# cartographer-project/cartographer

Hardware: AMD Instinct MI355X
Metric: candidate poses scored/sec (higher is better)
Workload: dtype u8/int32; 1 GPU; C2: 2D FastCorrelativeScanMatcher MatchFullSubmap (branch and bound): 1000-point scan vs 1 400x400 submap(s) per GPU, depth 7, full-angle search, m...; submaps_per_gpu=1, rotations=2373, found=1

## Files before the change

cartographer_amd/csrc/cmx_common.h:

```cpp
#ifndef CMX_COMMON_H_
#define CMX_COMMON_H_

#include <hip/hip_runtime.h>

#include <cstdarg>
#include <cstdint>
#include <cstdio>
#include <cstring>
#include <functional>
#include <mutex>
#include <string>
#include <vector>

#include "../../include/cartographer_mi355x.h"

namespace cmx {

void SetLastError(const char* fmt, ...);
const char* LastError();

struct HipError {
  cmx_status status;
};

#define CMX_HIP(expr)                                                              \
  do {                                                                             \
    hipError_t cmx_err__ = (expr);                                                 \
    if (cmx_err__ != hipSuccess) {                                                 \
      ::cmx::SetLastError("%s failed: %s (%s:%d)", #expr,                          \
                          hipGetErrorString(cmx_err__), __FILE__, __LINE__);       \
      throw ::cmx::HipError{cmx_err__ == hipErrorOutOfMemory ? CMX_OUT_OF_MEMORY   \
                                                             : CMX_DEVICE_ERROR};  \
    }                                                                              \
  } while (0)

#define CMX_REQUIRE(cond, ...)                       \
  do {                                               \
    if (!(cond)) {                                   \
      ::cmx::SetLastError(__VA_ARGS__);              \
      throw ::cmx::HipError{CMX_INVALID_ARGUMENT};   \
    }                                                \
  } while (0)

template <typename F>
cmx_status Guard(F&& body) {
  try {
    body();
    return CMX_OK;
  } catch (const HipError& e) {
    return e.status;
  } catch (const std::bad_alloc&) {
    SetLastError("host allocation failed");
    return CMX_OUT_OF_MEMORY;
  } catch (const std::exception& e) {
    SetLastError("exception: %s", e.what());
    return CMX_DEVICE_ERROR;
  }
}

#define CMX_DEBUG_OPTIONS(X)                                                                      \
  X(rt2d_legacy)                 \
  X(rt2d_tile)                                        \
  X(rt2d_groups)                                   \
  X(rt2d_target)                                    \
  X(rt2d_lds_kb)                                         \
  X(rt2d_no_image_cache)             \
  X(rt2d_parts)                                 \
  X(rt2d_host_par)         \
  X(rt2d_tables_serial)    \
  X(rt2d_first_part)       \
  X(rt2d_image_kernels)    \
  X(rt2d_no_lane)          \
  X(rt2d_parts_pool)       \
  X(rt2d_grid_share)       \
  X(rt2d_unfused)            \
  X(rt2d_no_bounds)        \
  X(rt2d_bounds)           \
  X(rt2d_bounds_fused)     \
  X(rt2d_bounds_level)     \
  X(rt2d_bounds_verify)    \
  X(rt2d_tsdf_batch_legacy)  \
  X(rt2d_tsdf_batch_bulk)  \
  X(rt2d_tsdf_verify)      \
  X(timeline)                  \
  X(trace)                       \
  X(host_trace)                          \
  X(launch_serial)         \
  X(sync)                      \
  X(no_copy_kernels)             \
  X(timing)                \
  X(no_direct_results)     \
  X(frontier_capacity)     \
  X(comm_virtual_ranks)    \
  X(comm_force_rccl)       \
  X(fast2d_unfused)                    \
  X(fast2d_store_scans)                   \
  X(fast2d_fused_threads)                            \
  X(fast2d_fanout)         \
  X(fast2d_group)          \
  X(fast2d_group_verify)   \
  X(fast2d_levels_per_stage)                                    \
  X(fast2d_wave_levels)                        \
  X(fast2d_xcd_affinity)                          \
  X(fast2d_dive)           \
  X(fast2d_queue)          \
  X(fast2d_queue_blocks)                \
  X(fast2d_queue_capacity)              \
  X(fast2d_queue_lost)       \
  X(filters_generic)       \
  X(fast3d_byte_loads)                             \
  X(fast3d_affinity)                              \
  X(fast3d_no_families)                             \
  X(fast3d_no_oct)                                         \
  X(fast3d_batch)                                                 \
  X(fast3d_chunk_cells)    \
  X(rt3d_legacy)                  \
  X(rt3d_no_tiles)                      \
  X(rt3d_verify)                  \
  X(rt3d_no_rotblocks)              \
  X(rt3d_rotblock_permille)  \
  X(rt3d_crosscheck)           \
  X(rt3d_expand_all)       \
  X(rt3d_unstaged)                                     \
  X(rt3d_no_boxes)                            \
  X(rt3d_report)                                             \
  X(rt3d_segments)                         \
  X(rt3d_group_rotations)                                  \
  X(rt3d_group_tile_kb)                                   \
  X(rt3d_group_float)                          \
  X(rt3d_cand_threads)                                   \
  X(rt3d_cand_rotations)                                    \
  X(rt3d_cand_tile_kb)
struct DebugOptions {
#define CMX_DEBUG_FIELD(name) int name = 0;
  CMX_DEBUG_OPTIONS(CMX_DEBUG_FIELD)
#undef CMX_DEBUG_FIELD
};
const DebugOptions& Debug();
bool DebugSet(const char* name, int value);

void UseDevice(int device);

void ParallelFor(int n, int serial_below, const std::function<void(int)>& fn);

class LaunchTurn {
 public:
  LaunchTurn();
  ~LaunchTurn();
  LaunchTurn(const LaunchTurn&) = delete;
  LaunchTurn& operator=(const LaunchTurn&) = delete;
 private:
  bool held_;
};

class HostLane {
 public:
  HostLane();
  ~HostLane();
  HostLane(const HostLane&) = delete;
  HostLane& operator=(const HostLane&) = delete;
  void Run(std::function<void()> fn);
  void Wait();
  bool own() const { return own_; }

 private:
  bool own_ = false, pending_ = false;
};

class DeviceBuffer {
 public:
  DeviceBuffer() = default;
  DeviceBuffer(const DeviceBuffer&) = delete;
  DeviceBuffer& operator=(const DeviceBuffer&) = delete;
  ~DeviceBuffer() { Free(); }
  void* Reserve(size_t bytes) {
    if (bytes > capacity_) {
      Free();
      const size_t want = bytes + bytes / 4 + 256;
      CMX_HIP(hipMalloc(&ptr_, want));
      capacity_ = want;
    }
    return ptr_;
  }
  template <typename T>
  T* ReserveAs(size_t count) { return static_cast<T*>(Reserve(count * sizeof(T))); }
  void* get() const { return ptr_; }
  size_t capacity() const { return capacity_; }
// ... 131 lines not shown
```

cartographer_amd/csrc/fast_2d.hip:

```cpp
#include <algorithm>
#include <chrono>
#include <cstring>
#include <memory>
#include <type_traits>
#include <utility>

#include "fast_2d_device.h"
#include "fast_2d_internal.h"

namespace cmx {
namespace {

constexpr int kSeedsPerProblem = 64;

constexpr int kMaxStages = kMaxDepth + 2;

constexpr int kCountStride = 32;
constexpr int kQueues = 2048;
struct alignas(8) QueueCtl {
  int head;
  int reserved;
  int pad[30];
};
struct Counters {
  int frontier[kMaxStages][kSubLists * kCountStride];
  int leaves[kSubLists * kCountStride];
  int frontier_overflow;
  int leaf_overflow;
  unsigned wave_gathers;
  int blocks_done;
  int pad[28];
  unsigned gathers_shard[16 * kCountStride];
  unsigned queue_stats[16 * kCountStride];
  QueueCtl queue[kQueues];
};

struct CountersSummary {
  int leaves[kSubLists];
  int frontier_total[kMaxStages];
  int frontier_overflow;
  int leaf_overflow;
  unsigned wave_gathers;
  int pad;
  unsigned queue_stats[8];
};

struct NodeList {
  Node2D* nodes;
  int* counts;
  int sub_capacity;
};

__device__ __forceinline__ int ListReserve(const NodeList& list, int sub, int m) {
  return atomicAdd(&list.counts[sub * kCountStride], m);
}
__device__ __forceinline__ bool ListStore(const NodeList& list, int sub, int slot,
                                          const Node2D& nd) {
  if (slot >= list.sub_capacity) return false;
  list.nodes[static_cast<size_t>(sub) * list.sub_capacity + slot] = nd;
  return true;
}
__device__ __forceinline__ int ListMaxCount(const NodeList& list) {
  const int lane = threadIdx.x & 63;
  return WaveMax(min(list.counts[lane * kCountStride], list.sub_capacity));
}

__device__ __forceinline__ int NodeProblem(const Node2D& nd) { return nd.problem & 0xffffff; }
__device__ __forceinline__ int NodeLevel(const Node2D& nd) { return nd.problem >> 24; }

__device__ __forceinline__ Node2D CoarseNode(const Fast2DProblem& P, int problem, int s,
                                             int local) {
  const int2 dims = P.coarse_dims[s];
  const int4 bd = P.bounds[s];
  const int step = 1 << (P.depth - 1);
  const int ix = local / dims.y, iy = local - ix * dims.y;
  const int c = s * P.coarse_stride + local;
  Node2D nd;
  nd.problem = problem | ((P.depth - 1) << 24);
  nd.scan = s;
  nd.dx = bd.x + ix * step;
  nd.dy = bd.z + iy * step;
  nd.score = P.coarse_score[c];
  nd.coarse_index = c;
  nd.path = 0;
  nd.coarse_score = nd.score;
  return nd;
}

struct SeedScratch {
  int hist[1024];
  int wave_total[4];
  int threshold_bin;
  int found_scan[4];
  int total;
};

__device__ __forceinline__ void PickSeeds(const Fast2DProblem& P, int n, int want0, int wants,
                                          SeedScratch* sh) {
  const int tid = threadIdx.x, lane = tid & 63, T = blockDim.x;
  for (int i = tid; i < 1024; i += T) sh->hist[i] = 0;
  if (tid < 4) sh->found_scan[tid] = -1;
  if (tid == 0) sh->total = 0;
  __syncthreads();
  const int S = P.num_scans;
  const long long range = 255ll * n + 1;
  const auto* scan_best = AsGlobal(P.scan_best);
  const auto* coarse_dims = AsGlobal(P.coarse_dims);
  const bool grouped = P.group > 1;
  const auto best_of = [&](int s) -> int {
    if (grouped) {
      const int first = s - s % kFusedGroup;
      if (s != first + (S - first >= kFusedGroup ? 1 : 0)) return -1;
    }
    return scan_best[s].x;
  };
  constexpr int kOwn = 16;
  int own[kOwn];
#pragma unroll
  for (int k = 0; k < kOwn; ++k) {
    const int s = tid + k * T;
    own[k] = s < S ? best_of(s) : -1;
  }
  int total = 0;
#pragma unroll
  for (int k = 0; k < kOwn; ++k)
    if (own[k] >= 0) atomicAdd(&sh->hist[static_cast<int>(own[k] * 1024ll / range)], 1);
  for (int s = tid + kOwn * T; s < S; s += T) {
    const int b = best_of(s);
    if (b >= 0) atomicAdd(&sh->hist[static_cast<int>(b * 1024ll / range)], 1);
  }
  if (want0 == 0) {
    for (int s = tid; s < S; s += T) total += coarse_dims[s].x * coarse_dims[s].y;
    total = WaveSum(total);
    if (lane == 0 && total) atomicAdd(&sh->total, total);
  }
  __syncthreads();
  if (tid < 64) {
    int mine = 0;
#pragma unroll
    for (int k = 0; k < 16; ++k) mine += sh->hist[1023 - 16 * lane - k];
    int incl = mine;
#pragma unroll
    for (int off = 1; off < 64; off <<= 1) {
      const int o = __shfl_up(incl, off, 64);
      if (lane >= off) incl += o;
    }
    const unsigned long long reached = __ballot(incl >= kSeedsPerProblem);
    int tb = 0;
    if (reached) {
      const int first = __ffsll(static_cast<long long>(reached)) - 1;
      if (lane == first) {
        int acc = incl - mine;
        for (int k = 0; k < 16; ++k) {
          const int b = 1023 - 16 * lane - k;
          acc += sh->hist[b];
          if (acc >= kSeedsPerProblem) { tb = b; break; }
        }
        sh->threshold_bin = tb;
      }
    } else if (lane == 0) {
      sh->threshold_bin = 0;
    }
  }
  __syncthreads();
  const int tb = sh->threshold_bin;
  const auto qualifies = [&](int best) {
    return best >= 0 && static_cast<int>(best * 1024ll / range) >= tb &&
           ToScore(P, best, n) > P.min_score;
  };
// ... 162 lines not shown
    const int total = sh->partial[0][k] + sh->partial[1][k] + sh->partial[2][k] + sh->partial[3][k];
    const float mine = valid ? ToScoreCtx(ctx, total) : -1.f;
    int rank = 0, nvalid = 0;
#pragma unroll
    for (int j = 0; j < 4; ++j) {
      const float other = __shfl(mine, j, 64);
      if (other >= 0.f) ++nvalid;
      if (j != k && other >= 0.f && (other > mine || (other == mine && j < k))) ++rank;
    }
    if (threadIdx.x < 4) {
      sh->child_score[k] = mine;
      sh->rank[k] = rank;
      if (k == 0) sh->nvalid = nvalid;
    }
  }
  __syncthreads();
}

__device__ __forceinline__ Node2D MakeChild(const Node2D& nd, int k, int child_level,
                                            const ChildScratch& sh) {
  Node2D child = nd;
  child.problem = NodeProblem(nd) | (child_level << 24);
  child.dx = nd.dx + (k >> 1) * (1 << child_level);
  child.dy = nd.dy + (k & 1) * (1 << child_level);
  child.score = sh.child_score[k];
  child.path = nd.path | (static_cast<unsigned>(sh.rank[k]) << (2 * child_level));
  return child;
}

__device__ __forceinline__ void RecordLeaf(const Node2D& leaf, const NodeList& leaves,
                                           Counters* __restrict__ counters) {
  const int sub = blockIdx.x & (kSubLists - 1);
  if (!ListStore(leaves, sub, ListReserve(leaves, sub, 1), leaf)) counters->leaf_overflow = 1;
}

__global__ void __launch_bounds__(256, 4)
DiveKernel(const Fast2DProblem* __restrict__ problems, ProblemState* __restrict__ states, int n,
           NodeList leaves, Counters* __restrict__ counters) {
  const int problem = blockIdx.y;
  const Fast2DProblem& P = problems[problem];
  ProblemState& st = states[problem];
  if (st.error) return;
  __shared__ BlockContext ctx;
  __shared__ ChildScratch sh;
  __shared__ Node2D cur;
  __shared__ SeedScratch seed_scratch;
  const int per_seed = P.group > 1 ? kFusedGroup : 1;
  if (static_cast<int>(blockIdx.x) >= kSeedsPerProblem * per_seed) return;
  int seed_scan;
  const bool have_seed = PickSeed(P, n, blockIdx.x / per_seed, &seed_scratch, &seed_scan);
  if (blockIdx.x == 0 && threadIdx.x == 0) st.coarse_total = seed_scratch.total;
  if (!have_seed) return;
  if (per_seed > 1) {
    seed_scan = seed_scan - seed_scan % kFusedGroup + static_cast<int>(blockIdx.x) % per_seed;
    if (seed_scan >= P.num_scans) return;
  }
  const Node2D seed = CoarseNode(P, problem, seed_scan, P.scan_best[seed_scan].y);
  if (threadIdx.x == 0) cur = seed;
  LoadContext(P, n, seed.scan, &ctx);
  const int depth = NodeLevel(seed) + 1;
  unsigned long long scored = 0;
  for (int child_level = depth - 2; child_level >= 0; --child_level) {
    const Node2D nd = cur;
    ScoreChildren(ctx, nd.dx, nd.dy, child_level, &sh);
    scored += sh.nvalid;
    if (threadIdx.x == 0) {
      for (int k = 0; k < 4; ++k)
        if (sh.child_score[k] >= 0.f && sh.rank[k] == 0) cur = MakeChild(nd, k, child_level, sh);
    }
    __syncthreads();
  }
  if (threadIdx.x == 0) {
    const Node2D leaf = cur;
    if (leaf.score > ctx.min_score) {
      RecordLeaf(leaf, leaves, counters);
      atomicMax(&st.best_bits, __float_as_uint(leaf.score));
    }
    atomicAdd(&st.scored_shard[blockIdx.x & (kStatShards - 1)], scored);
    atomicAdd(&st.expanded_shard[blockIdx.x & (kStatShards - 1)],
              static_cast<unsigned long long>(depth - 1));
  }
}

__global__ void __launch_bounds__(256)
FilterCoarseKernel(const Fast2DProblem* __restrict__ problems,
                   const ProblemState* __restrict__ states, int n, int chunk, int num_chunks,
                   int strict, int affinity, NodeList out, Counters* __restrict__ counters) {
  const int problem = blockIdx.y;
  const Fast2DProblem& P = problems[problem];
  const int lane = threadIdx.x & 63;
  const int s = blockIdx.x * 4 + __builtin_amdgcn_readfirstlane(threadIdx.x >> 6);
  if (s >= P.num_scans || states[problem].error) return;
  if (s % num_chunks != chunk) return;
  const float best = __uint_as_float(states[problem].best_bits);
  const float top = ToScore(P, P.scan_best[s].x, n);
  if (strict ? !(top > best) : (top < best)) return;
  const int2 dims = P.coarse_dims[s];
  const int count = dims.x * dims.y;
  const int base = s * P.coarse_stride;
  const auto* scores = AsGlobal(P.coarse_score) + base;
  float ahead[4];
#pragma unroll
  for (int k = 0; k < 4; ++k) ahead[k] = k * kWave + lane < count ? scores[k * kWave + lane] : 0.f;
  for (int c0 = 0; c0 < count; c0 += kWave) {
    const int sub = affinity ? (problem & 7) + 8 * ((s + (c0 >> 6)) & 7)
                             : (s + blockIdx.y + (c0 >> 6)) & (kSubLists - 1);
    const int c = c0 + lane;
    bool keep = false;
    if (c < count) {
      float score;
      switch (c0 >> 6) {
        case 0: score = ahead[0]; break;
        case 1: score = ahead[1]; break;
        case 2: score = ahead[2]; break;
        case 3: score = ahead[3]; break;
        default: score = scores[c];
      }
      keep = strict ? (score > best) : (score >= best);
    }
    const unsigned long long mask = __ballot(keep);
    if (mask == 0) continue;
    int first = 0;
    if (lane == 0) first = ListReserve(out, sub, __popcll(mask));
    first = __builtin_amdgcn_readfirstlane(first);
    if (keep) {
      const int slot = first + __popcll(mask & ((1ull << lane) - 1));
      if (!ListStore(out, sub, slot, CoarseNode(P, problem, s, c))) counters->frontier_overflow = 1;
    }
  }
}

constexpr int kWaveStatProblems = 1024;

__global__ void __launch_bounds__(256)
ExpandWaveKernel(const Fast2DProblem* __restrict__ problems, ProblemState* __restrict__ states,
                 int n, NodeList in, int strict, int affinity, NodeList out,
                 Counters* __restrict__ counters) {
  __shared__ unsigned stat_scored[kWaveStatProblems], stat_expanded[kWaveStatProblems];
  __shared__ unsigned stat_gathers;
  if (threadIdx.x == 0) stat_gathers = 0;
  for (int i = threadIdx.x; i < kWaveStatProblems; i += blockDim.x) {
    stat_scored[i] = 0;
    stat_expanded[i] = 0;
  }
  __syncthreads();
  const int lane = threadIdx.x & 63;
  const int wave = __builtin_amdgcn_readfirstlane(threadIdx.x >> 6);
  const int max_count = ListMaxCount(in);
  int first = blockIdx.x * 4 + wave;
  if (affinity) {
    const int slot = (blockIdx.x >> 3) * 4 + wave;
    first = (slot >> 3) * kSubLists + (blockIdx.x & 7) + 8 * (slot & 7);
  }
  const int out_sub = first & (kSubLists - 1);
  for (int i = first; i < max_count * kSubLists; i += gridDim.x * 4) {
    const int in_sub = i & (kSubLists - 1), j = i / kSubLists;
    if (j >= in.counts[in_sub * kCountStride]) continue;
    const Node2D nd = in.nodes[static_cast<size_t>(in_sub) * in.sub_capacity + j];
    const int problem = NodeProblem(nd);
    const Fast2DProblem& P = problems[problem];
    ProblemState& st = states[problem];
    const float best = __uint_as_float(st.best_bits);
    if (strict ? !(nd.score > best) : (nd.score < best)) continue;
    const int child_level = NodeLevel(nd) - 1;
    const LevelDesc L = P.level[child_level];
    const int4 bd = P.bounds[nd.scan];
    const int half = 1 << child_level, off = half - 1;
    const bool vx = nd.dx + half <= bd.y, vy = nd.dy + half <= bd.w;
    const auto* pts = AsGlobal(P.discrete) + static_cast<size_t>(nd.scan) * n;
    const bool recompute = P.recompute_scans != 0 && P.store_scans == 0;
    const float2 rot = recompute ? P.scan_rot[nd.scan] : make_float2(1.f, 0.f);
    const int parent_ub = SumUpperBound(P, nd.score, n);
    const unsigned long long quad_bytes =
        static_cast<unsigned long long>((L.qy + 3) >> 2) * static_cast<unsigned>(L.qtx) * 128ull;
    const bool quads_by_buffer = quad_bytes < (1ull << 31);
    const __amdgpu_buffer_rsrc_t quad_rsrc = __builtin_amdgcn_make_buffer_rsrc(
        const_cast<uint32_t*>(L.quads), 0, quads_by_buffer ? static_cast<int>(quad_bytes) : 0,
        0x00020000);
    const auto* quads = AsGlobal(L.quads);
    const uint32_t child_mask =
        (vx ? 0xffffffffu : 0x0000ffffu) & (vy ? 0xffffffffu : 0x00ff00ffu);
    int s00 = 0, s01 = 0, s10 = 0, s11 = 0, seen_max = 0;
    int groups = 0;
    bool dead = false;
    constexpr int kIters = 4;
    constexpr int kGroup = kIters * kWave;
    const auto walk = [&](auto recompute_tag, auto buffer_tag) {
      constexpr bool kRecompute = decltype(recompute_tag)::value;
      constexpr bool kBuffer = decltype(buffer_tag)::value;
      for (int q0 = 0; q0 < n; q0 += kGroup) {
        uint32_t cell[kIters];
#pragma unroll
        for (int u = 0; u < kIters; ++u) {
          const int q = q0 + u * kWave + lane;
          const int at = q < n ? q : 0;
          if constexpr (kRecompute) cell[u] = ScanCell(P, rot, at);
          else cell[u] = pts[at];
        }
        uint32_t v[kIters];
#pragma unroll
        for (int u = 0; u < kIters; ++u) {
          const int q = q0 + u * kWave + lane;
          const bool live = q < n;
          const uint32_t p = cell[u];
          const int X = static_cast<short>(p & 0xffffu) + nd.dx + off + half;
          const int Y = static_cast<short>(p >> 16) + nd.dy + off + half;
          const bool inside = live && static_cast<unsigned>(X) < static_cast<unsigned>(L.qx) &&
                              static_cast<unsigned>(Y) < static_cast<unsigned>(L.qy);
          if constexpr (kBuffer) {
            const uint32_t quad = __builtin_amdgcn_raw_buffer_load_b32(
                quad_rsrc, inside ? QuadOffset(X, Y, L.qtx) * 4u : 0xfffffff0u, 0, 0);
            v[u] = quad & child_mask;
// ... 546 lines not shown
  const int lane = threadIdx.x & 63;
  const auto* pts = AsGlobal(P.discrete) + static_cast<size_t>(scan) * n;
  if constexpr (kRecompute) {
    const float2 rot = P.scan_rot[scan];
#pragma unroll
    for (int u = 0; u < kChainCells; ++u) cell[u] = kNoCell;
#pragma unroll 1
    for (int j = 0; j * kWave < n; ++j) {
      const int i = j * kWave + lane;
      const uint32_t c = i < n ? ScanCell(P, rot, i) : kNoCell;
#pragma unroll
      for (int u = 0; u < kChainCells; ++u) cell[u] = u == j ? c : cell[u];
    }
  } else {
#pragma unroll
    for (int j = 0; j < kChainCells; ++j) {
      const int i = j * kWave + lane;
      cell[j] = kNoCell;
      if (j * kWave < n) cell[j] = i < n ? pts[i] : kNoCell;
    }
  }
}

struct ChainLevel {
  int qx, qy, qtx;
  int half;
  int ax, ay;
  __amdgpu_buffer_rsrc_t quad_rsrc;
};

__device__ __forceinline__ ChainLevel MakeChainLevel(const Fast2DProblem& P, int child_level,
                                                     int dx, int dy) {
  const LevelDesc& Lm = P.level[child_level];
  ChainLevel L;
  L.half = 1 << child_level;
  L.ax = dx + 2 * L.half - 1;
  L.ay = dy + 2 * L.half - 1;
  L.qx = __builtin_amdgcn_readfirstlane(Lm.qx);
  L.qy = __builtin_amdgcn_readfirstlane(Lm.qy);
  L.qtx = __builtin_amdgcn_readfirstlane(Lm.qtx);
  const unsigned long long quads_address = reinterpret_cast<unsigned long long>(Lm.quads);
  const unsigned long long quads_uniform =
      static_cast<unsigned long long>(static_cast<unsigned>(
          __builtin_amdgcn_readfirstlane(static_cast<unsigned>(quads_address)))) |
      (static_cast<unsigned long long>(static_cast<unsigned>(
           __builtin_amdgcn_readfirstlane(static_cast<unsigned>(quads_address >> 32)))) << 32);
  const unsigned long long quad_bytes =
      static_cast<unsigned long long>((L.qy + 3) >> 2) * static_cast<unsigned>(L.qtx) * 128ull;
  L.quad_rsrc = __builtin_amdgcn_make_buffer_rsrc(
      reinterpret_cast<uint32_t*>(quads_uniform), 0, static_cast<int>(quad_bytes), 0x00020000);
  return L;
}

template <int kFirst, int kCount, bool kWantMax>
__device__ __forceinline__ void ChainGather(const ChainLevel& L, const uint32_t (&cell)[kChainCells],
                                            uint32_t* even, uint32_t* odd, int* seen_max) {
  typedef unsigned short Halves __attribute__((ext_vector_type(2)));
  uint32_t v[kCount];
#pragma unroll
  for (int u = 0; u < kCount; ++u) {
    const uint32_t p = cell[kFirst + u];
    const unsigned X = static_cast<unsigned>(static_cast<short>(p & 0xffffu) + L.ax);
    const unsigned Y = static_cast<unsigned>(static_cast<short>(p >> 16) + L.ay);
    const bool inside = X < static_cast<unsigned>(L.qx) && Y < static_cast<unsigned>(L.qy);
    const unsigned tile = __umul24(Y >> 2, static_cast<unsigned>(L.qtx)) + (X >> 3);
    const unsigned byte = (tile << 7) | ((Y & 3u) << 5) | ((X & 7u) << 2);
    v[u] = __builtin_amdgcn_raw_buffer_load_b32(L.quad_rsrc, inside ? byte : 0xfffffff0u, 0, 0);
  }
#pragma unroll
  for (int u = 0; u < kCount; ++u) {
    const uint32_t e = v[u] & 0x00ff00ffu, o = (v[u] >> 8) & 0x00ff00ffu;
    *even += e;
    *odd += o;
    if constexpr (kWantMax) {
      Halves eh, oh;
      __builtin_memcpy(&eh, &e, 4);
      __builtin_memcpy(&oh, &o, 4);
      const Halves m = __builtin_elementwise_max(eh, oh);
      *seen_max += static_cast<int>(max(m.x, m.y));
    }
  }
}

__global__ void __launch_bounds__(256)
DiveWaveKernel(const Fast2DProblem* __restrict__ problems, ProblemState* __restrict__ states, int n,
               NodeList leaves, Counters* __restrict__ counters) {
  const int problem = blockIdx.y;
  const Fast2DProblem& P = problems[problem];
  ProblemState& st = states[problem];
  if (st.error) return;
  __shared__ SeedScratch seed_scratch;
  const bool grouped = P.group > 1;
  const int seeds = grouped ? 1 : 4;
  const int want0 = static_cast<int>(blockIdx.x) * seeds;
  if (want0 >= kSeedsPerProblem) return;
  PickSeeds(P, n, want0, seeds, &seed_scratch);
  if (blockIdx.x == 0 && threadIdx.x == 0) st.coarse_total = seed_scratch.total;
  const int lane = threadIdx.x & 63;
  const int wave = __builtin_amdgcn_readfirstlane(threadIdx.x >> 6);
  if (grouped && wave >= kFusedGroup) return;
  int seed_scan = __builtin_amdgcn_readfirstlane(seed_scratch.found_scan[grouped ? 0 : wave]);
  if (seed_scan < 0) return;
  if (grouped) {
    seed_scan = seed_scan - seed_scan % kFusedGroup + wave;
    if (seed_scan >= P.num_scans) return;
  }
  const Node2D seed = CoarseNode(P, problem, seed_scan, P.scan_best[seed_scan].y);
  uint32_t cell[kChainCells];
  const bool stored =
      !P.recompute_scans ||
      (P.store_scans && !(ToScore(P, P.scan_best[seed_scan].x, n) < fmaxf(P.min_score, 0.f)));
  if (__builtin_amdgcn_readfirstlane(stored ? 1 : 0)) LoadChainCells<false>(P, n, seed_scan, cell);
  else LoadChainCells<true>(P, n, seed_scan, cell);
  const int4 bd = P.bounds[seed_scan];
  const int depth = P.depth;
  int dx = __builtin_amdgcn_readfirstlane(seed.dx), dy = __builtin_amdgcn_readfirstlane(seed.dy);
  float score = seed.score;
  unsigned long long scored = 0;
  for (int child_level = depth - 2; child_level >= 0; --child_level) {
    const ChainLevel L = MakeChainLevel(P, child_level, dx, dy);
    const bool vx = dx + L.half <= bd.y, vy = dy + L.half <= bd.w;
    uint32_t even = 0, odd = 0;
    if (n > 8 * kWave) ChainGather<0, 16, false>(L, cell, &even, &odd, nullptr);
    else if (n > 4 * kWave) ChainGather<0, 8, false>(L, cell, &even, &odd, nullptr);
    else ChainGather<0, 4, false>(L, cell, &even, &odd, nullptr);
    const int total[4] = {WaveSum(static_cast<int>(even & 0xffffu)), WaveSum(static_cast<int>(odd & 0xffffu)),
                          WaveSum(static_cast<int>(even >> 16)), WaveSum(static_cast<int>(odd >> 16))};
    int kbest = 0, nvalid = 0;
    float best_score = -1.f;
#pragma unroll
    for (int k = 0; k < 4; ++k) {
      const bool valid = ((k >> 1) == 0 || vx) && ((k & 1) == 0 || vy);
      const float sc = valid ? ToScore(P, total[k], n) : -1.f;
      nvalid += valid ? 1 : 0;
      if (sc >= 0.f && (k == 0 || sc > best_score)) { kbest = k; best_score = sc; }
    }
    kbest = __builtin_amdgcn_readfirstlane(kbest);
    dx += (kbest >> 1) * L.half;
    dy += (kbest & 1) * L.half;
    score = best_score;
    scored += nvalid;
  }
  if (lane == 0) {
    if (score > P.min_score) {
      Node2D leaf = seed;
      leaf.problem = problem;
      leaf.dx = dx;
      leaf.dy = dy;
      leaf.score = score;
      RecordLeaf(leaf, leaves, counters);
      atomicMax(&st.best_bits, __float_as_uint(score));
    }
    const int shard = (blockIdx.x * 4 + wave) & (kStatShards - 1);
    atomicAdd(&st.scored_shard[shard], scored);
    atomicAdd(&st.expanded_shard[shard], static_cast<unsigned long long>(depth - 1));
  }
}

__device__ __forceinline__ void RecordLeafAgent(const Node2D& leaf, const NodeList& leaves,
                                                int sub, Counters* __restrict__ counters) {
  const int slot = ListReserve(leaves, sub, 1);
  if (slot >= leaves.sub_capacity) {
    __hip_atomic_store(&counters->leaf_overflow, 1, __ATOMIC_RELAXED, __HIP_MEMORY_SCOPE_AGENT);
    return;
  }
  unsigned long long v[4];
  __builtin_memcpy(v, &leaf, sizeof(Node2D));
  unsigned long long* at = reinterpret_cast<unsigned long long*>(
      &leaves.nodes[static_cast<size_t>(sub) * leaves.sub_capacity + slot]);
#pragma unroll
  for (int k = 0; k < 4; ++k)
    __hip_atomic_store(&at[k], v[k], __ATOMIC_RELAXED, __HIP_MEMORY_SCOPE_AGENT);
}

__global__ void __launch_bounds__(256)
TreeQueueKernel(const Fast2DProblem* __restrict__ problems, ProblemState* __restrict__ states, int n,
                NodeList in, TreeQueue Q, NodeList leaves, Counters* __restrict__ counters,
                SelectState* __restrict__ sel, BestLeaf* __restrict__ best_out, int num_problems,
                ProblemState* __restrict__ states_out, CountersSummary* __restrict__ summary,
                const unsigned* __restrict__ tail_dev, unsigned* __restrict__ tail_host,
                int tail_words, int counters_trace, int max_lost) {
  static_assert(sizeof(Node2D) == 32, "a node is eight words: eight granules, four leaf stores");
  const int lane = threadIdx.x & 63;
  const int wave_id = blockIdx.x * 4 + __builtin_amdgcn_readfirstlane(threadIdx.x >> 6);
  const int num_waves = gridDim.x * 4;
  const int queues = min(num_waves, kQueues);
  const int home = wave_id % queues;
  unsigned steals = 0;
  unsigned long long scored = 0, expanded = 0;
  unsigned gathers = 0;
  unsigned q_pops = 0, q_lost = 0, q_rereads = 0, q_pushed = 0, q_listed = 0, q_chains = 0;
  int stat_problem = -1;
  const auto flush_stats = [&]() {
    if (lane == 0 && stat_problem >= 0 && expanded) {
      ProblemState& st = states[stat_problem];
      atomicAdd(&st.scored_shard[wave_id & (kStatShards - 1)], scored);
      atomicAdd(&st.expanded_shard[wave_id & (kStatShards - 1)], expanded);
    }
    scored = expanded = 0;
  };
  const int in_slots = ListMaxCount(in) * kSubLists;
  int round = 0;
  Node2D mine{};
  unsigned mine_bits = 0;
  bool round_loaded = false, share_done = false;
  bool pushed_any = false;
  Node2D nd;
  for (;;) {
    bool have = false;
    while (!have && !share_done) {
      if (!round_loaded) {
        if (wave_id + static_cast<long long>(round) * 64 * num_waves >= in_slots) { share_done = true; break; }
        const long long i = wave_id + (static_cast<long long>(round) * 64 + lane) * num_waves;
        ++round;
        mine_bits = 0;
        if (i < in_slots) {
          const int in_sub = static_cast<int>(i & (kSubLists - 1)), j = static_cast<int>(i / kSubLists);
          if (j < min(in.counts[in_sub * kCountStride], in.sub_capacity)) {
            mine = in.nodes[static_cast<size_t>(in_sub) * in.sub_capacity + j];
            mine_bits = max(__float_as_uint(fmaxf(mine.score, 0.f)), 1u);
          }
        }
        round_loaded = true;
      }
      const unsigned top = static_cast<unsigned>(WaveMax(static_cast<int>(mine_bits)));
      const float bound_now = __uint_as_float(LoadAgent(&states[0].best_bits));
      if (top == 0 || (num_problems == 1 && __uint_as_float(top) < bound_now)) {
        round_loaded = false;
        continue;
      }
      const int l = __ffsll(static_cast<long long>(__ballot(mine_bits == top))) - 1;
      nd.problem = __builtin_amdgcn_readlane(mine.problem, l);
      nd.scan = __builtin_amdgcn_readlane(mine.scan, l);
      nd.dx = __builtin_amdgcn_readlane(mine.dx, l);
      nd.dy = __builtin_amdgcn_readlane(mine.dy, l);
      nd.score = __uint_as_float(__builtin_amdgcn_readlane(__float_as_uint(mine.score), l));
      nd.coarse_index = __builtin_amdgcn_readlane(mine.coarse_index, l);
      nd.path = __builtin_amdgcn_readlane(mine.path, l);
// ... 242 lines not shown

  Workspace& ws;
  const PreparedBatch& batch;
  BatchResult* result;
  const int num, n, depth;
  int frontier_capacity, frontier_sub;
  Node2D* d_front[2] = {nullptr, nullptr};
  NodeList leaf_list;
  Counters* d_counters;
  SearchTail d_tail, h_tail;
  bool direct;
  int strict = 0;
  int num_chunks = 1;
};

SearchRun::SearchRun(Workspace& ws, const PreparedBatch& batch, BatchResult* result)
    : ws(ws), batch(batch), result(result), num(batch.num_problems), n(batch.n),
      depth(batch.h_problems[0].depth) {
  const auto capacity = [](int v, int fallback) {
    return v >= kSubLists ? std::min(v, fallback) / kSubLists * kSubLists : fallback;
  };
  const int frontier_default = static_cast<int>(
      std::min<long long>(1ll << 25, std::max<long long>(1ll << 21, 65536ll * num)));
  frontier_capacity = capacity(Debug().frontier_capacity, frontier_default);
  frontier_sub = frontier_capacity / kSubLists;
  const int leaf_capacity = capacity(0, 1 << 20);
  Node2D* d_leaves = ws.dev[12].ReserveAs<Node2D>(leaf_capacity);
  d_counters = reinterpret_cast<Counters*>(batch.d_misc);
  d_tail = SearchTail(batch.d_misc + sizeof(Counters), num);
  leaf_list = NodeList{d_leaves, d_counters->leaves, leaf_capacity / kSubLists};
  h_tail = SearchTail(static_cast<char*>(ws.pinned[3].Reserve(SearchTail::Bytes(num))), num);
  direct = Debug().no_direct_results == 0 && h_tail.bytes % sizeof(unsigned) == 0;
}

void SearchRun::FetchResults(bool published) {
  if (!published)
    SmallCopyAsync(h_tail.base, d_tail.base, h_tail.bytes, false, ws.stream);
  const auto t0 = std::chrono::steady_clock::now();
  CMX_HIP(hipStreamSynchronize(ws.stream));
  g_host_wait_ns += std::chrono::duration_cast<std::chrono::nanoseconds>(
                        std::chrono::steady_clock::now() - t0).count();
}

void SearchRun::PrepareStrictRetry() {
  CMX_REQUIRE(num_chunks < (1 << 12), "branch-and-bound overflow not resolvable");
  if (h_tail.summary->frontier_overflow) num_chunks *= 4;
  strict = 1;
  for (int p = 0; p < num; ++p) {
    const float floor_score = std::max(batch.h_problems[p].min_score, 0.f);
    unsigned floor_bits;
    std::memcpy(&floor_bits, &floor_score, sizeof(float));
    if (h_tail.states[p].best_bits > floor_bits) h_tail.states[p].best_bits -= 1;
  }
  CMX_HIP(hipMemcpyAsync(batch.d_states, h_tail.states, num * sizeof(ProblemState),
                         hipMemcpyHostToDevice, ws.stream));
  CMX_HIP(hipMemsetAsync(d_counters, 0, sizeof(Counters), ws.stream));
}

void RunDepthOne(SearchRun& run) {
  Workspace& ws = run.ws;
  SelectDepthOneKernel<<<run.num, 1024, 0, ws.stream>>>(
      run.batch.d_problems, run.batch.d_states, run.n, run.d_tail.best, run.d_tail.states);
  CMX_HIP(hipGetLastError());
  RecordEvent(ws.ev_end, ws.stream);
  run.FetchResults(false);
}

bool ChainWalkPossible(const SearchRun& run) {
  bool chain_ok = run.n <= kChainCells * kWave;
  for (const Fast2DProblem& P : run.batch.h_problems)
    for (int l = 0; l + 1 < run.depth; ++l)
      chain_ok = chain_ok && static_cast<unsigned long long>((P.level[l].qy + 3) >> 2) *
                                     static_cast<unsigned>(P.level[l].qtx) * 128ull < (1ull << 31);
  return chain_ok;
}

bool QueueSearchPossible(const SearchRun& run) {
  bool queue_ok = QueueSearchWanted(run.n, run.num) && ChainWalkPossible(run);
  for (const Fast2DProblem& P : run.batch.h_problems)
    queue_ok = queue_ok && (P.recompute_scans == 0 || P.store_scans != 0);
  return queue_ok;
}

enum class QueueOutcome { kDone, kLeafOverflow, kQueueOverflow };

QueueOutcome RunQueueSearch(SearchRun& run, std::unique_ptr<LaunchTurn> turn) {
  Workspace& ws = run.ws;
  const PreparedBatch& batch = run.batch;
  BatchResult* result = run.result;
  const int num = run.num, n = run.n;
  const long long wanted = std::max<long long>(1ll << 20, 65536ll * num);
  int sub_capacity = static_cast<int>(std::min<long long>(wanted, 1ll << 23) / kQueues);
  if (Debug().fast2d_queue_capacity > 0) sub_capacity = Debug().fast2d_queue_capacity;
  TreeQueue queue;
  queue.capacity = sub_capacity;
  queue.slots = static_cast<unsigned long long*>(ws.tagged[0].Acquire(
      static_cast<size_t>(kQueues) * sub_capacity * 8 * sizeof(unsigned long long), ws.stream,
      &queue.epoch));
  run.d_front[0] = ws.dev[10].ReserveAs<Node2D>(run.frontier_capacity);
  FilterCoarseKernel<<<dim3(DivUp(batch.max_scans, 4), num), 256, 0, ws.stream>>>(
      batch.d_problems, batch.d_states, n, 0, 1, 0, 0, run.Front(0),
      run.d_counters);
  run.Mark("filter");
  RecordEvent(ws.ev_x0, ws.stream);
  const int blocks = Debug().fast2d_queue_blocks > 0
                         ? Debug().fast2d_queue_blocks
                         : std::min(2048, 256 * std::max(1, (num + 3) / 4));
  TreeQueueKernel<<<blocks, 256, 0, ws.stream>>>(
      batch.d_problems, batch.d_states, n, run.Front(0), queue, run.leaf_list, run.d_counters,
      run.d_tail.sel, run.d_tail.best, num, run.d_tail.states, run.d_tail.summary,
      run.d_tail.words(), run.PublishTo(), run.h_tail.num_words(),
      batch.trace && batch.trace->enabled() ? 1 : 0,
      Debug().fast2d_queue_lost > 0 ? Debug().fast2d_queue_lost : 3);
  run.Mark("queue");
  CMX_HIP(hipGetLastError());
  RecordEvent(ws.ev_x1, ws.stream);
  result->expansion_launches = 1;
  RecordEvent(ws.ev_end, ws.stream);
  turn.reset();
  run.FetchResults(run.direct);
  const CountersSummary& h_counters = *run.h_tail.summary;
  result->expansion_lookups = 64ll * h_counters.wave_gathers;
  for (int p = 0; p < num; ++p)
    for (int k = 0; k < kStatShards; ++k)
      result->expansion_nodes += run.h_tail.states[p].expanded_shard[k];
  if (h_counters.leaf_overflow) return QueueOutcome::kLeafOverflow;
  if (h_counters.frontier_overflow) return QueueOutcome::kQueueOverflow;
  return QueueOutcome::kDone;
}

void RunLevelSynchronous(SearchRun& run) {
  Workspace& ws = run.ws;
  const PreparedBatch& batch = run.batch;
  BatchResult* result = run.result;
  const int num = run.num, n = run.n;
  const CountersSummary& h_counters = *run.h_tail.summary;
  const int kLevelsPerStage = std::max(0, Debug().fast2d_levels_per_stage);
  const int kWaveLevels = Debug().fast2d_wave_levels > 0 ? Debug().fast2d_wave_levels - 1 : -1;
  const int levels_per_stage = kLevelsPerStage > 0 ? kLevelsPerStage : (num < 4 ? kMaxDepth : 2);
  const int wave_levels = kWaveLevels >= 0 ? kWaveLevels : (num < 4 ? 1 : 2);
  const int affinity_override = Debug().fast2d_xcd_affinity;
  const int affinity = affinity_override ? affinity_override - 1 : (num >= 16 ? 1 : 0);
  const int wide_blocks = std::min(4096, 1024 * std::max(1, (num + 3) / 4));
  const int narrow_blocks = std::min(4096, 512 * std::max(1, (num + 3) / 4));
  run.d_front[0] = ws.dev[10].ReserveAs<Node2D>(run.frontier_capacity);
  run.d_front[1] = ws.dev[11].ReserveAs<Node2D>(run.frontier_capacity);
  for (;;) {
    const int strict = run.strict;
    for (int chunk = 0; chunk < run.num_chunks; ++chunk) {
      if (chunk > 0 || strict)
        CMX_HIP(hipMemsetAsync(run.d_counters->frontier, 0, sizeof(run.d_counters->frontier),
                               ws.stream));
      FilterCoarseKernel<<<dim3(DivUp(batch.max_scans, 4), num), 256, 0, ws.stream>>>(
          batch.d_problems, batch.d_states, n, chunk, run.num_chunks, strict, affinity,
          run.Front(0), run.d_counters);
      run.Mark("filter");
      int stage = 0;
      int top = run.depth - 1;
      const bool timed = !strict && chunk == 0 && num >= 4;
      if (timed) RecordEvent(ws.ev_x0, ws.stream);
      for (int used = 0; used < wave_levels && top - 1 >= 1; ++used, --top, ++stage) {
        ExpandWaveKernel<<<used == 0 ? wide_blocks : narrow_blocks, 256, 0, ws.stream>>>(
            batch.d_problems, batch.d_states, n, run.Front(stage), strict, affinity,
            run.Front(stage + 1), run.d_counters);
        run.Mark("wave");
      }
      if (timed) {
        RecordEvent(ws.ev_x1, ws.stream);
        result->expansion_launches = stage;
      }
      for (; top > 0; top -= levels_per_stage, ++stage) {
        const int stop = std::max(0, top - levels_per_stage);
        SubtreeKernel<<<narrow_blocks, 256, 0, ws.stream>>>(
            batch.d_problems, batch.d_states, n, run.Front(stage), stop, strict,
            run.Front(stage + 1), run.leaf_list, run.d_counters);
        run.Mark("subtree");
      }
    }
    SelectBestKernel<<<1, 1024, 0, ws.stream>>>(
        run.leaf_list, batch.d_states, run.d_tail.sel, run.d_tail.best, num, run.d_tail.states,
        run.d_counters, run.d_tail.summary, run.d_tail.words(), run.PublishTo(),
        run.h_tail.num_words());
    run.Mark("select");
    CMX_HIP(hipGetLastError());
    RecordEvent(ws.ev_end, ws.stream);
    run.FetchResults(run.direct);
    if (!strict) {
      for (int st = 0; st < result->expansion_launches; ++st)
        result->expansion_nodes += h_counters.frontier_total[st];
      result->expansion_lookups = 64ll * h_counters.wave_gathers;
    }
    if (!h_counters.frontier_overflow && !h_counters.leaf_overflow) break;
    run.PrepareStrictRetry();
  }
}

void TraceListSizes(const CountersSummary& h_counters) {
  fprintf(stderr, "[cmx trace] list sizes:");
  for (int st = 0; st < kMaxStages; ++st)
    if (h_counters.frontier_total[st])
      fprintf(stderr, " frontier[%d]=%d", st, h_counters.frontier_total[st]);
  long long leaves = 0;
  for (int k = 0; k < kSubLists; ++k) leaves += h_counters.leaves[k];
  fprintf(stderr, " leaves=%lld\n", leaves);
  const unsigned* q = h_counters.queue_stats;
  if (q[5])
    fprintf(stderr, "[cmx trace] work queue: %u chains (%u nodes from the list, %u popped), %u "
            "pushed, %u lost races, %u slot re-reads\n", q[5], q[4], q[0], q[3], q[1], q[2]);
}

}

bool QueueSearchWanted(int n, int num) {
  return Debug().fast2d_queue != 2 && n <= kChainCells * kWave && (num < 4 || Debug().fast2d_queue == 1);
}

void ReserveSearchScratch(Workspace& ws, int num, PreparedBatch* batch) {
  batch->d_misc = static_cast<char*>(ws.dev[14].Reserve(SearchMiscBytes(num)));
  batch->num_counter_words = static_cast<int>(sizeof(Counters) / sizeof(int));
}

thread_local long long g_host_wait_ns = 0;

void RunBranchAndBound(Workspace& ws, const PreparedBatch& batch, BatchResult* result) {
  const int num = batch.num_problems;
  const int depth = batch.h_problems[0].depth;
  for (const Fast2DProblem& P : batch.h_problems)
    CMX_REQUIRE(P.depth == depth, "all matchers of a batch must share branch_and_bound_depth");
  SearchRun run(ws, batch, result);
  if (depth == 1) {
    RunDepthOne(run);
  } else {
    std::unique_ptr<LaunchTurn> turn(new LaunchTurn);
    if (Debug().fast2d_dive != 1 && ChainWalkPossible(run)) {
      DiveWaveKernel<<<dim3(batch.any_group ? kSeedsPerProblem : kSeedsPerProblem / 4, num), 256, 0,
                       ws.stream>>>(batch.d_problems, batch.d_states, run.n, run.leaf_list,
                                    run.d_counters);
    } else {
      DiveKernel<<<dim3(kSeedsPerProblem * (batch.any_group ? kFusedGroup : 1), num), 256, 0, ws.stream>>>(
          batch.d_problems, batch.d_states, run.n, run.leaf_list, run.d_counters);
    }
    run.Mark("seed+dive");
    bool searched = false;
    if (QueueSearchPossible(run)) {
      switch (RunQueueSearch(run, std::move(turn))) {
        case QueueOutcome::kDone:
          searched = true;
          break;
        case QueueOutcome::kLeafOverflow:
          run.PrepareStrictRetry();
          break;
        case QueueOutcome::kQueueOverflow:
          CMX_HIP(hipMemsetAsync(run.d_counters, 0, sizeof(Counters), ws.stream));
          break;
      }
    }
    turn.reset();
    if (!searched) RunLevelSynchronous(run);
  }

  result->best.assign(run.h_tail.best, run.h_tail.best + num);
  result->states.assign(run.h_tail.states, run.h_tail.states + num);
  if (depth > 1) {
    if (batch.trace && batch.trace->enabled()) TraceListSizes(*run.h_tail.summary);
    result->d_leaves = run.leaf_list.nodes;
    result->leaf_sub_capacity = run.leaf_list.sub_capacity;
    result->leaf_counts.assign(run.h_tail.summary->leaves, run.h_tail.summary->leaves + kSubLists);
  }
  result->device_ms = ElapsedMs(ws.ev_begin, ws.ev_end);
  result->dominant_ms = ElapsedMs(ws.ev_k0, ws.ev_k1);
  if (result->expansion_launches > 0) result->expansion_ms = ElapsedMs(ws.ev_x0, ws.ev_x1);
}

}
```

Baseline: 10.71 billion candidates/s.

## Fold coarse frontier filtering into the wave dive kernel

Moves the coarse-level filter that seeds the tree queue into the tail of DiveWaveKernel, so each block filters a strided subset of rotations after its dive finishes. This removes a separate kernel launch and can use the best score found during the dive to prune rotations. Each wave batches up to four surviving rotations, issuing the score loads and list reservations together. In exchange the dive kernel does more work on its small grid (16 blocks for one problem), which may give less parallelism than the old dedicated filter launch. The filter always uses non-strict comparison and non-affinity sublist placement.

```diff
diff --git a/cartographer_amd/csrc/cmx_common.h b/cartographer_amd/csrc/cmx_common.h
--- a/cartographer_amd/csrc/cmx_common.h
+++ b/cartographer_amd/csrc/cmx_common.h
@@ -103,6 +103,7 @@
   X(fast2d_wave_levels)                        \
   X(fast2d_xcd_affinity)                          \
   X(fast2d_dive)           \
+  X(fast2d_fold_filter)    \
   X(fast2d_queue)          \
   X(fast2d_queue_blocks)                \
   X(fast2d_queue_capacity)              \
diff --git a/cartographer_amd/csrc/fast_2d.hip b/cartographer_amd/csrc/fast_2d.hip
--- a/cartographer_amd/csrc/fast_2d.hip
+++ b/cartographer_amd/csrc/fast_2d.hip
@@ -68,10 +68,8 @@
 __device__ __forceinline__ int NodeProblem(const Node2D& nd) { return nd.problem & 0xffffff; }
 __device__ __forceinline__ int NodeLevel(const Node2D& nd) { return nd.problem >> 24; }
 
-__device__ __forceinline__ Node2D CoarseNode(const Fast2DProblem& P, int problem, int s,
-                                             int local) {
-  const int2 dims = P.coarse_dims[s];
-  const int4 bd = P.bounds[s];
+__device__ __forceinline__ Node2D CoarseNodeOf(const Fast2DProblem& P, int problem, int s,
+                                               int local, int2 dims, int4 bd, float score) {
   const int step = 1 << (P.depth - 1);
   const int ix = local / dims.y, iy = local - ix * dims.y;
   const int c = s * P.coarse_stride + local;
@@ -80,11 +78,17 @@
   nd.scan = s;
   nd.dx = bd.x + ix * step;
   nd.dy = bd.z + iy * step;
-  nd.score = P.coarse_score[c];
+  nd.score = score;
   nd.coarse_index = c;
   nd.path = 0;
-  nd.coarse_score = nd.score;
+  nd.coarse_score = score;
   return nd;
+}
+
+__device__ __forceinline__ Node2D CoarseNode(const Fast2DProblem& P, int problem, int s,
+                                             int local) {
+  return CoarseNodeOf(P, problem, s, local, P.coarse_dims[s], P.bounds[s],
+                      P.coarse_score[s * P.coarse_stride + local]);
 }
 
 struct SeedScratch {
@@ -413,52 +417,92 @@
   }
 }
 
+template <int K>
+__device__ __forceinline__ void FilterRotations(const Fast2DProblem& P, int problem,
+                                                const int (&s)[K], const int2 (&dims)[K],
+                                                const int4 (&bd)[K], int live, float best,
+                                                int strict, int affinity, const NodeList& out,
+                                                Counters* __restrict__ counters) {
+  const int lane = threadIdx.x & 63;
+  const auto* all_scores = AsGlobal(P.coarse_score);
+  const auto sub_of = [&](int scan, int run) {
+    return affinity ? (problem & 7) + 8 * ((scan + run) & 7)
+                    : (scan + problem + run) & (kSubLists - 1);
+  };
+  const auto kept = [&](float score) { return strict ? (score > best) : (score >= best); };
+  int count[K];
+  float ahead[K][4];
+#pragma unroll
+  for (int k = 0; k < K; ++k) {
+    count[k] = k < live ? dims[k].x * dims[k].y : 0;
+    const auto* scores = all_scores + s[k] * P.coarse_stride;
+#pragma unroll
+    for (int j = 0; j < 4; ++j)
+      ahead[k][j] = j * kWave + lane < count[k] ? scores[j * kWave + lane] : 0.f;
+  }
+  unsigned long long mask[K][4];
+  int first[K][4];
+#pragma unroll
+  for (int k = 0; k < K; ++k) {
+#pragma unroll
+    for (int j = 0; j < 4; ++j) {
+      mask[k][j] = __ballot(j * kWave + lane < count[k] && kept(ahead[k][j]));
+      first[k][j] = 0;
+      if (lane == 0 && mask[k][j])
+        first[k][j] = ListReserve(out, sub_of(s[k], j), __popcll(mask[k][j]));
+    }
+  }
+#pragma unroll
+  for (int k = 0; k < K; ++k) {
+#pragma unroll
+    for (int j = 0; j < 4; ++j) {
+      if (mask[k][j] == 0) continue;
+      const int slot0 = __builtin_amdgcn_readfirstlane(first[k][j]);
+      if ((mask[k][j] >> lane) & 1ull) {
+        const int slot = slot0 + __popcll(mask[k][j] & ((1ull << lane) - 1));
+        if (!ListStore(out, sub_of(s[k], j), slot,
+                       CoarseNodeOf(P, problem, s[k], j * kWave + lane, dims[k], bd[k], ahead[k][j])))
+          counters->frontier_overflow = 1;
+      }
+    }
+  }
+#pragma unroll
+  for (int k = 0; k < K; ++k) {
+    const auto* scores = all_scores + s[k] * P.coarse_stride;
+    for (int c0 = 4 * kWave; c0 < count[k]; c0 += kWave) {
+      const int c = c0 + lane;
+      const float score = c < count[k] ? scores[c] : 0.f;
+      const unsigned long long more = __ballot(c < count[k] && kept(score));
+      if (more == 0) continue;
+      const int sub = sub_of(s[k], c0 >> 6);
+      int slot0 = 0;
+      if (lane == 0) slot0 = ListReserve(out, sub, __popcll(more));
+      slot0 = __builtin_amdgcn_readfirstlane(slot0);
+      if ((more >> lane) & 1ull) {
+        const int slot = slot0 + __popcll(more & ((1ull << lane) - 1));
+        if (!ListStore(out, sub, slot, CoarseNodeOf(P, problem, s[k], c, dims[k], bd[k], score)))
+          counters->frontier_overflow = 1;
+      }
+    }
+  }
+}
+
 __global__ void __launch_bounds__(256)
 FilterCoarseKernel(const Fast2DProblem* __restrict__ problems,
                    const ProblemState* __restrict__ states, int n, int chunk, int num_chunks,
                    int strict, int affinity, NodeList out, Counters* __restrict__ counters) {
   const int problem = blockIdx.y;
   const Fast2DProblem& P = problems[problem];
-  const int lane = threadIdx.x & 63;
   const int s = blockIdx.x * 4 + __builtin_amdgcn_readfirstlane(threadIdx.x >> 6);
   if (s >= P.num_scans || states[problem].error) return;
   if (s % num_chunks != chunk) return;
   const float best = __uint_as_float(states[problem].best_bits);
   const float top = ToScore(P, P.scan_best[s].x, n);
   if (strict ? !(top > best) : (top < best)) return;
-  const int2 dims = P.coarse_dims[s];
-  const int count = dims.x * dims.y;
-  const int base = s * P.coarse_stride;
-  const auto* scores = AsGlobal(P.coarse_score) + base;
-  float ahead[4];
-#pragma unroll
-  for (int k = 0; k < 4; ++k) ahead[k] = k * kWave + lane < count ? scores[k * kWave + lane] : 0.f;
-  for (int c0 = 0; c0 < count; c0 += kWave) {
-    const int sub = affinity ? (problem & 7) + 8 * ((s + (c0 >> 6)) & 7)
-                             : (s + blockIdx.y + (c0 >> 6)) & (kSubLists - 1);
-    const int c = c0 + lane;
-    bool keep = false;
-    if (c < count) {
-      float score;
-      switch (c0 >> 6) {
-        case 0: score = ahead[0]; break;
-        case 1: score = ahead[1]; break;
-        case 2: score = ahead[2]; break;
-        case 3: score = ahead[3]; break;
-        default: score = scores[c];
-      }
-      keep = strict ? (score > best) : (score >= best);
-    }
-    const unsigned long long mask = __ballot(keep);
-    if (mask == 0) continue;
-    int first = 0;
-    if (lane == 0) first = ListReserve(out, sub, __popcll(mask));
-    first = __builtin_amdgcn_readfirstlane(first);
-    if (keep) {
-      const int slot = first + __popcll(mask & ((1ull << lane) - 1));
-      if (!ListStore(out, sub, slot, CoarseNode(P, problem, s, c))) counters->frontier_overflow = 1;
-    }
-  }
+  const int rotation[1] = {s};
+  const int2 dims[1] = {P.coarse_dims[s]};
+  const int4 bd[1] = {P.bounds[s]};
+  FilterRotations<1>(P, problem, rotation, dims, bd, 1, best, strict, affinity, out, counters);
 }
 
 constexpr int kWaveStatProblems = 1024;
@@ -1171,29 +1215,10 @@
   }
 }
 
-__global__ void __launch_bounds__(256)
-DiveWaveKernel(const Fast2DProblem* __restrict__ problems, ProblemState* __restrict__ states, int n,
-               NodeList leaves, Counters* __restrict__ counters) {
-  const int problem = blockIdx.y;
-  const Fast2DProblem& P = problems[problem];
-  ProblemState& st = states[problem];
-  if (st.error) return;
-  __shared__ SeedScratch seed_scratch;
-  const bool grouped = P.group > 1;
-  const int seeds = grouped ? 1 : 4;
-  const int want0 = static_cast<int>(blockIdx.x) * seeds;
-  if (want0 >= kSeedsPerProblem) return;
-  PickSeeds(P, n, want0, seeds, &seed_scratch);
-  if (blockIdx.x == 0 && threadIdx.x == 0) st.coarse_total = seed_scratch.total;
+__device__ __forceinline__ void WaveDive(const Fast2DProblem& P, ProblemState& st, int problem,
+                                         int n, int seed_scan, int wave, const NodeList& leaves,
+                                         Counters* __restrict__ counters) {
   const int lane = threadIdx.x & 63;
-  const int wave = __builtin_amdgcn_readfirstlane(threadIdx.x >> 6);
-  if (grouped && wave >= kFusedGroup) return;
-  int seed_scan = __builtin_amdgcn_readfirstlane(seed_scratch.found_scan[grouped ? 0 : wave]);
-  if (seed_scan < 0) return;
-  if (grouped) {
-    seed_scan = seed_scan - seed_scan % kFusedGroup + wave;
-    if (seed_scan >= P.num_scans) return;
-  }
   const Node2D seed = CoarseNode(P, problem, seed_scan, P.scan_best[seed_scan].y);
   uint32_t cell[kChainCells];
   const bool stored =
@@ -1243,6 +1268,78 @@
     const int shard = (blockIdx.x * 4 + wave) & (kStatShards - 1);
     atomicAdd(&st.scored_shard[shard], scored);
     atomicAdd(&st.expanded_shard[shard], static_cast<unsigned long long>(depth - 1));
+  }
+}
+
+template <bool kFold>
+__global__ void __launch_bounds__(256)
+DiveWaveKernel(const Fast2DProblem* __restrict__ problems, ProblemState* __restrict__ states, int n,
+               NodeList leaves, NodeList front, Counters* __restrict__ counters) {
+  const int problem = blockIdx.y;
+  const Fast2DProblem& P = problems[problem];
+  ProblemState& st = states[problem];
+  if (st.error) return;
+  __shared__ SeedScratch seed_scratch;
+  const bool grouped = P.group > 1;
+  const int seeds = grouped ? 1 : 4;
+  const int want0 = static_cast<int>(blockIdx.x) * seeds;
+  const int lane = threadIdx.x & 63;
+  const int wave = __builtin_amdgcn_readfirstlane(threadIdx.x >> 6);
+  int seed_scan = -1;
+  if (want0 < kSeedsPerProblem) {
+    PickSeeds(P, n, want0, seeds, &seed_scratch);
+    if (blockIdx.x == 0 && threadIdx.x == 0) st.coarse_total = seed_scratch.total;
+    if (!grouped || wave < kFusedGroup) {
+      seed_scan = __builtin_amdgcn_readfirstlane(seed_scratch.found_scan[grouped ? 0 : wave]);
+      if (seed_scan >= 0 && grouped) {
+        seed_scan = seed_scan - seed_scan % kFusedGroup + wave;
+        if (seed_scan >= P.num_scans) seed_scan = -1;
+      }
+    }
+  }
+  if (seed_scan >= 0) WaveDive(P, st, problem, n, seed_scan, wave, leaves, counters);
+  if constexpr (kFold) {
+    asm volatile("s_waitcnt vmcnt(0)" ::: "memory");
+    __syncthreads();
+    const int S = P.num_scans;
+    const int G = gridDim.x;
+    const auto* scan_best = AsGlobal(P.scan_best);
+    constexpr int kAtOnce = 4;
+    const auto* coarse_dims = AsGlobal(P.coarse_dims);
+    const auto* bounds = AsGlobal(P.bounds);
+    for (int i0 = wave; static_cast<int>(blockIdx.x) + static_cast<long long>(i0) * G < S;
+         i0 += 4 * kWave) {
+      const long long s_long = static_cast<int>(blockIdx.x) + static_cast<long long>(i0 + 4 * lane) * G;
+      const bool exists = s_long < S;
+      const int s_mine = exists ? static_cast<int>(s_long) : 0;
+      const int top_mine = exists ? scan_best[s_mine].x : 0;
+      const int2 dims_mine = make_int2(exists ? coarse_dims[s_mine].x : 0,
+                                       exists ? coarse_dims[s_mine].y : 0);
+      const int4 bd_mine = make_int4(exists ? bounds[s_mine].x : 0, 0,
+                                     exists ? bounds[s_mine].z : 0, 0);
+      const float bound = __uint_as_float(LoadAgent(&st.best_bits));
+      unsigned long long alive = __ballot(exists && !(ToScore(P, top_mine, n) < bound));
+      while (alive) {
+        int rotation[kAtOnce];
+        int2 dims[kAtOnce];
+        int4 bd[kAtOnce];
+        int live = 0;
+#pragma unroll
+        for (int k = 0; k < kAtOnce; ++k) {
+          const int l = alive ? __ffsll(static_cast<long long>(alive)) - 1 : 0;
+          live += alive ? 1 : 0;
+          alive &= alive - 1;
+          rotation[k] = __builtin_amdgcn_readlane(s_mine, l);
+          dims[k] = make_int2(__builtin_amdgcn_readlane(dims_mine.x, l),
+                              __builtin_amdgcn_readlane(dims_mine.y, l));
+          bd[k] = make_int4(__builtin_amdgcn_readlane(bd_mine.x, l), 0,
+                            __builtin_amdgcn_readlane(bd_mine.z, l), 0);
+        }
+        FilterRotations<kAtOnce>(P, problem, rotation, dims, bd, live,
+                                 __uint_as_float(LoadAgent(&st.best_bits)), 0,
+                                 0, front, counters);
+      }
+    }
   }
 }
 
@@ -1651,14 +1748,9 @@
   return queue_ok;
 }
 
-enum class QueueOutcome { kDone, kLeafOverflow, kQueueOverflow };
-
-QueueOutcome RunQueueSearch(SearchRun& run, std::unique_ptr<LaunchTurn> turn) {
+TreeQueue ReserveQueueSearch(SearchRun& run) {
   Workspace& ws = run.ws;
-  const PreparedBatch& batch = run.batch;
-  BatchResult* result = run.result;
-  const int num = run.num, n = run.n;
-  const long long wanted = std::max<long long>(1ll << 20, 65536ll * num);
+  const long long wanted = std::max<long long>(1ll << 20, 65536ll * run.num);
   int sub_capacity = static_cast<int>(std::min<long long>(wanted, 1ll << 23) / kQueues);
   if (Debug().fast2d_queue_capacity > 0) sub_capacity = Debug().fast2d_queue_capacity;
   TreeQueue queue;
@@ -1667,10 +1759,23 @@
       static_cast<size_t>(kQueues) * sub_capacity * 8 * sizeof(unsigned long long), ws.stream,
       &queue.epoch));
   run.d_front[0] = ws.dev[10].ReserveAs<Node2D>(run.frontier_capacity);
-  FilterCoarseKernel<<<dim3(DivUp(batch.max_scans, 4), num), 256, 0, ws.stream>>>(
-      batch.d_problems, batch.d_states, n, 0, 1, 0, 0, run.Front(0),
-      run.d_counters);
-  run.Mark("filter");
+  return queue;
+}
+
+enum class QueueOutcome { kDone, kLeafOverflow, kQueueOverflow };
+
+QueueOutcome RunQueueSearch(SearchRun& run, const TreeQueue& queue, bool filtered,
+                            std::unique_ptr<LaunchTurn> turn) {
+  Workspace& ws = run.ws;
+  const PreparedBatch& batch = run.batch;
+  BatchResult* result = run.result;
+  const int num = run.num, n = run.n;
+  if (!filtered) {
+    FilterCoarseKernel<<<dim3(DivUp(batch.max_scans, 4), num), 256, 0, ws.stream>>>(
+        batch.d_problems, batch.d_states, n, 0, 1, 0, 0, run.Front(0),
+        run.d_counters);
+    run.Mark("filter");
+  }
   RecordEvent(ws.ev_x0, ws.stream);
   const int blocks = Debug().fast2d_queue_blocks > 0
                          ? Debug().fast2d_queue_blocks
@@ -1800,19 +1905,29 @@
   if (depth == 1) {
     RunDepthOne(run);
   } else {
+    const bool wave_dive = Debug().fast2d_dive != 1 && ChainWalkPossible(run);
+    const bool queue_search = QueueSearchPossible(run);
+    const bool fold = queue_search && wave_dive && Debug().fast2d_fold_filter == 0;
+    TreeQueue queue{};
+    if (queue_search) queue = ReserveQueueSearch(run);
     std::unique_ptr<LaunchTurn> turn(new LaunchTurn);
-    if (Debug().fast2d_dive != 1 && ChainWalkPossible(run)) {
-      DiveWaveKernel<<<dim3(batch.any_group ? kSeedsPerProblem : kSeedsPerProblem / 4, num), 256, 0,
-                       ws.stream>>>(batch.d_problems, batch.d_states, run.n, run.leaf_list,
-                                    run.d_counters);
+    if (wave_dive) {
+      const dim3 grid(batch.any_group ? kSeedsPerProblem : kSeedsPerProblem / 4, num);
+      if (fold) {
+        DiveWaveKernel<true><<<grid, 256, 0, ws.stream>>>(
+            batch.d_problems, batch.d_states, run.n, run.leaf_list, run.Front(0), run.d_counters);
+      } else {
+        DiveWaveKernel<false><<<grid, 256, 0, ws.stream>>>(
+            batch.d_problems, batch.d_states, run.n, run.leaf_list, NodeList{}, run.d_counters);
+      }
     } else {
       DiveKernel<<<dim3(kSeedsPerProblem * (batch.any_group ? kFusedGroup : 1), num), 256, 0, ws.stream>>>(
           batch.d_problems, batch.d_states, run.n, run.leaf_list, run.d_counters);
     }
     run.Mark("seed+dive");
     bool searched = false;
-    if (QueueSearchPossible(run)) {
-      switch (RunQueueSearch(run, std::move(turn))) {
+    if (queue_search) {
+      switch (RunQueueSearch(run, queue, fold, std::move(turn))) {
         case QueueOutcome::kDone:
           searched = true;
           break;
```

Result: slower. 10.20 billion candidates/s (-4.8%).
